# zhiqwang/demonet

Measured on AMD Instinct MI355X. Metric: images/sec ssdlite320_mobilenet_v3_large fp16 end-to-end incl. NMS, higher is better.
Workload: dtype fp16; 1 GPU; ssdlite320_mobilenet_v3_large fp16, batch 64 per GPU, 320x320 synthetic images, K=91, synthetic weights seed 0, post-process incl. per-class top-300 + hard NMS; global_batch=64, forwards_in_flight=3, parallelism=single GPU, input=NCHW fp32 in [0,1], device-resident

## Files before the change

demonet_amd/csrc/headfuse.hip:

```cpp
#include <algorithm>
#include <type_traits>

#include "common.h"
#include "post_math.h"

namespace {

constexpr int HF_P = 64;
constexpr int HF_RUNP = 128;
constexpr int HF_ZOFF = 4 * HF_RUNP * 16;
constexpr int HF_WOFF = HF_ZOFF + 64;
constexpr int HF_XS = HF_WOFF + 1024;
constexpr int HF_BS = 4 * HF_P * 16;
constexpr int HF_LDS = 2 * HF_XS + 4 * HF_BS;
constexpr int HF_NP = 2;
constexpr int hf_post_tabs(int nc0, int nc1) {
    const int t = 32 * (nc0 + nc1) * 4 + 3 * 256 * 4 + HF_NP * 256 * 4 + 256;
    return t > HF_LDS ? t : HF_LDS;
}
constexpr int hf_post_lds(int nc0, int nc1) { return hf_post_tabs(nc0, nc1) + (((nc0 + 3) & ~3) + ((nc1 + 3) & ~3)) * 4; }

typedef unsigned u32x4 __attribute__((ext_vector_type(4)));
typedef unsigned u32x8 __attribute__((ext_vector_type(8)));
typedef float f32x8 __attribute__((ext_vector_type(8)));
typedef float f32x4_a8 __attribute__((ext_vector_type(4), aligned(8)));
typedef unsigned u32x16 __attribute__((ext_vector_type(16)));
typedef const __attribute__((address_space(4))) u32x4* cp_u4;
typedef const __attribute__((address_space(4))) u32x16* cp_u16;

struct HfLevel {
    const half_t* x;
    const half_t* wd;
    const unsigned char* wslot;
    const half_t* wf[2];
    const float* bias[2];
    float* out[2];
    unsigned out_img_stride[2];
    int nc[2];
    int H, W, C, hw, m;
    int act;
    int tiles;
    int ct0;
    int aoff, aloc, sbase;
    int sm;
};
struct HfGroup {
    int count, xq;
    int start[9];
    long long* stamps;
    HeadPost post;
    HfLevel lv[8];
};
#ifdef DN_DEV_STAMPS
#define HF_T(var) const long long var = (long long)__builtin_amdgcn_s_memtime()
#else
#define HF_T(var)
#endif

__device__ __forceinline__ void hf_fma8(float (&acc)[8], const u32x4& x, const u32x4& w) {
#pragma unroll
    for (int i = 0; i < 4; ++i) {
        asm("v_fma_mix_f32 %0, %1, %2, %0 op_sel_hi:[1,1,0]" : "+v"(acc[2 * i]) : "v"(x[i]), "s"(w[i]));
        asm("v_fma_mix_f32 %0, %1, %2, %0 op_sel:[1,1,0] op_sel_hi:[1,1,0]" : "+v"(acc[2 * i + 1]) : "v"(x[i]), "s"(w[i]));
    }
}

__device__ __forceinline__ void hf_fma8v(float (&acc)[8], const u32x4& x, const u32x4& w) {
#pragma unroll
    for (int i = 0; i < 4; ++i) {
        asm("v_fma_mix_f32 %0, %1, %2, %0 op_sel_hi:[1,1,0]" : "+v"(acc[2 * i]) : "v"(x[i]), "v"(w[i]));
        asm("v_fma_mix_f32 %0, %1, %2, %0 op_sel:[1,1,0] op_sel_hi:[1,1,0]" : "+v"(acc[2 * i + 1]) : "v"(x[i]), "v"(w[i]));
    }
}

constexpr int HF_SM_BATCHES = 3;
constexpr int HF_SM_MAX_K = 4 * 8 * HF_SM_BATCHES;
static_assert(HF_SM_MAX_K == 96, "hf_softmax_scores covers 96 classes: change head_fused_post_supported's bound with it");
__device__ __forceinline__ void hf_softmax_scores(const HeadPost& P, const float* __restrict__ lg, const unsigned* __restrict__ rowoff, const unsigned* __restrict__ ranc,
                                                  const unsigned char* __restrict__ rpart, unsigned* __restrict__ lhist, const int nrows, const int img_first,
                                                  const int te, const int K, const int ccb) {
#pragma clang fp contract(off)
    const int Km1 = K - 1, sub = te & 3;
    char* const sbase = reinterpret_cast<char*>(P.scoresT);
    const unsigned step4 = 4u * (unsigned)P.A;
    for (int rb = 0; rb < nrows; rb += 64) {
        const int row = rb + (te >> 2);
        const bool valid = row < nrows;
        const float* rp = lg + (valid ? rowoff[row] : 0u);
        float mx = -INFINITY, sm = 0.f;
        float v[8 * HF_SM_BATCHES];
#pragma unroll
        for (int b = 0; b < HF_SM_BATCHES; ++b) {
#pragma unroll
            for (int u = 0; u < 8; ++u) v[8 * b + u] = rp[min(sub + 32 * b + 4 * u, K - 1)];
#pragma unroll
            for (int u = 0; u < 8; ++u) mx = fmaxf(mx, v[8 * b + u]);
        }
        mx = fmaxf(mx, __shfl_xor(mx, 1));
        mx = fmaxf(mx, __shfl_xor(mx, 2));
#pragma unroll
        for (int b = 0; b < HF_SM_BATCHES; ++b) {
#pragma unroll
            for (int u = 0; u < 8; ++u) v[8 * b + u] = pp_exp_nonpos(v[8 * b + u] - mx);
#pragma unroll
            for (int u = 0; u < 8; ++u)
                if (sub + 32 * b + 4 * u < K) sm += v[8 * b + u];
        }
        sm += __shfl_xor(sm, 1);
        sm += __shfl_xor(sm, 2);
        if (!valid) continue;
        const float rinv = pp_row_rcp(sm);
        int rw = row;
        asm volatile("" : "+v"(rw));
        const unsigned q = rpart[rw];
        const unsigned hb = q * 256u;
        const unsigned ob4 = (((unsigned)(img_first + (int)q) * (unsigned)Km1) * (unsigned)P.A + ranc[rw]) * 4u + (unsigned)(sub - 1) * step4;
#pragma unroll
        for (int b = 0; b < HF_SM_BATCHES; ++b)
#pragma unroll
            for (int u = 0; u < 8; ++u) {
                const int k = sub + 32 * b + 4 * u;
                if (k >= 1 && k < K) {
                    const float sc = pp_score(v[8 * b + u], rinv);
                    *reinterpret_cast<float*>(sbase + (unsigned)(ob4 + (unsigned)(8 * b + u) * 4u * step4)) = sc;
                    if (sc > P.score_thr) {
                        atomicAdd(&lhist[hb + (unsigned)pp_hist_bin(sc, P.hb0, P.nb)], 1u);
                        if (ccb >= 0) atomicAdd(&lhist[hb + (unsigned)(ccb + k - 1)], 1u);
                    }
                }
            }
    }
}

template <int TCW, bool SM>
__global__ __launch_bounds__(256, 2) void head_fused_kernel(HfGroup g) {
    extern __shared__ __attribute__((aligned(16))) unsigned char hf_lds[];
    int p = 0;
#pragma unroll
    for (int i = 1; i < 8; ++i)
        if (i < g.count && (int)blockIdx.x >= g.start[i]) p = i;
    const HfLevel& L = g.lv[p];
    const int flat = blockIdx.x - g.start[p];
    int m0, mend;
    if (g.xq > 0 && L.tiles > 0) {
        const int grp = flat & 7, t = flat >> 3;
        const int r0 = grp * g.xq * L.hw;
        mend = min(L.m, r0 + g.xq * L.hw);
        m0 = r0 + t * HF_P;
    } else {
        m0 = flat * HF_P;
        mend = L.m;
    }
    if (m0 >= mend) return;

    const int tid = threadIdx.x, lane = tid & 63;
    const int wave = __builtin_amdgcn_readfirstlane(tid >> 6);
    const int r = lane & 31, hh = lane >> 5;
    const int C = L.C, W = L.W, H = L.H;
    const int NCH = C >> 5;

    unsigned tap3[3] = {0u, 0u, 0u};
    {
        const int mp = min(m0 + lane, mend - 1);
        const int img = mp / L.hw, rem = mp - img * L.hw;
        const int y = rem / W, x = rem - y * W;
#pragma unroll
        for (int ky = 0; ky < 3; ++ky)
#pragma unroll
            for (int kx = 0; kx < 3; ++kx) {
                const int iy = y + ky - 1, ix = x + kx - 1;
                const bool ok = iy >= 0 && iy < H && ix >= 0 && ix < W;
                const int P = lane + (W + 1) + (ky - 1) * W + (kx - 1);
                const unsigned slot = ok ? (unsigned)(4 * P + (wave ^ ((P >> 2) & 3))) : (unsigned)(HF_ZOFF / 16);
                tap3[ky] |= slot << (10 * kx);
            }
    }
    auto tap_addr = [&](int t) -> unsigned { return ((tap3[t / 3] >> (10 * (t % 3))) & 1023u) * 16u; };
    unsigned xoff[2];
#pragma unroll
    for (int i = 0; i < 2; ++i) {
        const int P = (2 * wave + i) * 16 + (lane >> 2);
        const int mp = min(max(m0 - (W + 1) + P, 0), L.m - 1);
        xoff[i] = ((unsigned)mp * (unsigned)C + (unsigned)(((lane & 3) ^ ((P >> 2) & 3)) * 8)) * 2u;
    }
    if (tid < 8) *reinterpret_cast<unsigned*>(hf_lds + (tid >> 2) * HF_XS + HF_ZOFF + (tid & 3) * 4) = 0u;
    const unsigned lds0 = (unsigned)(size_t)(__attribute__((address_space(3))) unsigned char*)hf_lds;
    auto glds16 = [&](const void* gsrc, unsigned dst) {
        unsigned keep;
        asm volatile("s_mov_b32 %0, m0\n\ts_mov_b32 m0, %2\n\ts_nop 0\n\tglobal_load_lds_dwordx4 %1, off\n\ts_mov_b32 m0, %0"
                     : "=&s"(keep) : "v"(gsrc), "s"(dst) : "memory");
    };
    const unsigned aoff = (unsigned)lane * 16u;
    const unsigned char* const xbase = reinterpret_cast<const unsigned char*>(L.x);
    auto stage_x = [&](int c) {
        const unsigned dst = lds0 + (c & 1) * HF_XS;
        glds16(xbase + (xoff[0] + (unsigned)c * 64u), dst + wave * 2048);
        glds16(xbase + (xoff[1] + (unsigned)c * 64u), dst + wave * 2048 + 1024);
        if (wave == 3) glds16(L.wslot + ((unsigned)c * 1024u + aoff), dst + HF_WOFF);
    };

    const int tlast = wave + 4 * (TCW - 1);
    const bool last_reg = tlast == L.ct0, last_on = tlast <= L.ct0;
    const int KS = C >> 4;
    const __amdgpu_buffer_rsrc_t ars0 = __builtin_amdgcn_make_buffer_rsrc(const_cast<half_t*>(L.wf[0]), 0, L.ct0 * KS * 1024, 0x00020000);
    const __amdgpu_buffer_rsrc_t ars1 = __builtin_amdgcn_make_buffer_rsrc(const_cast<half_t*>(L.wf[1]), 0, KS * 1024, 0x00020000);
    unsigned atile[TCW];
#pragma unroll
    for (int i = 0; i < TCW; ++i) {
        const int t = wave + 4 * i;
        const bool reg = (i == TCW - 1) && last_reg;
        atile[i] = reg ? 0u : (unsigned)(min(t, L.ct0 - 1) * KS) * 1024u;
    }
    auto load_a = [&](int i, int kstep) -> half8 {
        const u32x4 v = ((i == TCW - 1) && last_reg) ? __builtin_amdgcn_raw_buffer_load_b128(ars1, aoff, atile[i] + (unsigned)kstep * 1024u, 0)
                                                     : __builtin_amdgcn_raw_buffer_load_b128(ars0, aoff, atile[i] + (unsigned)kstep * 1024u, 0);
        return __builtin_bit_cast(half8, v);
    };
    const unsigned blast = last_reg ? (unsigned)HF_BS : 0u;

    floatx16 acc[TCW][2];
#pragma unroll
    for (int i = 0; i < TCW; ++i)
#pragma unroll
        for (int j = 0; j < 2; ++j)
#pragma unroll
            for (int e = 0; e < 16; ++e) acc[i][j][e] = 0.f;

    u32x16 w0a, w0b;
    u32x4 w0c;
    auto load_w0 = [&](int c) {
        const unsigned char* wp = reinterpret_cast<const unsigned char*>(L.wd) + (size_t)(c * 4 + wave) * 144;
        w0a = *(cp_u16)(wp);
        w0b = *(cp_u16)(wp + 64);
        w0c = *(cp_u4)(wp + 128);
    };
    auto w0tap = [&](int t) -> u32x4 {
        u32x4 r;
#pragma unroll
        for (int e = 0; e < 4; ++e) { const int d = 4 * t + e; r[e] = d < 16 ? w0a[d] : (d < 32 ? w0b[d - 16] : w0c[d - 32]); }
        return r;
    };

#ifdef DN_DEV_STAMPS
    long long st_dw = 0, st_wait = 0, st_mm = 0;
    const long long st_begin = (long long)__builtin_amdgcn_s_memtime();
    const long long st_begin_rt = (long long)__builtin_amdgcn_s_memrealtime();
#endif
    if constexpr (SM) if (L.sm) {
        float* const lb = reinterpret_cast<float*>(hf_lds + hf_post_tabs(L.nc[0], L.nc[1]));
        const int p0 = (L.nc[0] + 3) & ~3;
        for (int i = tid; i < L.nc[0]; i += 256) lb[i] = L.bias[0][i];
        if (tid < L.nc[1]) lb[p0 + tid] = L.bias[1][tid];
    }
    stage_x(0);
    load_w0(0);
    asm volatile("s_waitcnt vmcnt(0)" ::: "memory");
    __syncthreads();
    HF_T(st_loop);

    unsigned char* const bb = hf_lds + 2 * HF_XS;
    for (int c = 0; c < NCH; ++c) {
        const int PAR = c & 1;
        HF_T(st0);
        half8 af0[TCW], af1[TCW];
#pragma unroll
        for (int i = 0; i < TCW; ++i) af0[i] = load_a(i, 2 * c);
        {
            const unsigned char* xb = hf_lds + PAR * HF_XS;
            const unsigned char* wb = xb + HF_WOFF + wave * 144;
            asm volatile("" : "+v"(tap3[0]), "+v"(tap3[1]), "+v"(tap3[2]));
            const float4 bl4 = *reinterpret_cast<const float4*>(xb + HF_WOFF + 576 + wave * 32);
            const float4 bh4 = *reinterpret_cast<const float4*>(xb + HF_WOFF + 576 + wave * 32 + 16);
            const float4 cl4 = *reinterpret_cast<const float4*>(xb + HF_WOFF + 704 + wave * 32);
            const float4 ch4 = *reinterpret_cast<const float4*>(xb + HF_WOFF + 704 + wave * 32 + 16);
            float a0[8] = {cl4.x, cl4.y, cl4.z, cl4.w, ch4.x, ch4.y, ch4.z, ch4.w}, a1[8] = {bl4.x, bl4.y, bl4.z, bl4.w, bh4.x, bh4.y, bh4.z, bh4.w};
#pragma unroll
            for (int ky = 0; ky < 3; ++ky) {
                u32x4 tap[3], wv[3];
#pragma unroll
                for (int kx = 0; kx < 3; ++kx) {
                    tap[kx] = *reinterpret_cast<const u32x4*>(xb + tap_addr(ky * 3 + kx));
                    wv[kx] = *reinterpret_cast<const u32x4*>(wb + (ky * 3 + kx) * 16);
                }
                if (ky == 0 && c + 1 < NCH) stage_x(c + 1);
#pragma unroll
                for (int kx = 0; kx < 3; ++kx) hf_fma8(a0, tap[kx], w0tap(ky * 3 + kx));
                if (ky == 2) {
#pragma unroll
                    for (int i = 0; i < TCW; ++i) af1[i] = load_a(i, 2 * c + 1);
                }
#pragma unroll
                for (int kx = 0; kx < 3; ++kx) hf_fma8v(a1, tap[kx], wv[kx]);
                __builtin_amdgcn_sched_barrier(0);
            }
            unsigned char* bout = bb + PAR * 2 * HF_BS + wave * (HF_P * 16) + lane * 16;
            half8 o0, o1;
#pragma unroll
            for (int e = 0; e < 8; ++e) { o0[e] = (half_t)dn_relu6(a0[e]); o1[e] = (half_t)dn_relu6(a1[e]); }
            *reinterpret_cast<half8*>(bout) = o0;
            *reinterpret_cast<half8*>(bout + HF_BS) = o1;
        }
        HF_T(st1);
        asm volatile("s_waitcnt vmcnt(%0)" :: "n"(TCW) : "memory");
        __syncthreads();
        HF_T(st2);
        load_w0(min(c + 1, NCH - 1));
        {
            const unsigned char* bc = bb + PAR * 2 * HF_BS;
#pragma unroll
            for (int s = 0; s < 2; ++s) {
                half8 bf[2];
#pragma unroll
                for (int j = 0; j < 2; ++j) bf[j] = *reinterpret_cast<const half8*>(bc + (unsigned)((2 * s + hh) * (HF_P * 16) + (32 * j + r) * 16));
#pragma unroll
                for (int i = 0; i < TCW - 1; ++i)
#pragma unroll
                    for (int j = 0; j < 2; ++j) acc[i][j] = __builtin_amdgcn_mfma_f32_32x32x16_f16(s ? af1[i] : af0[i], bf[j], acc[i][j], 0, 0, 0);
                if (last_on) {
#pragma unroll
                    for (int j = 0; j < 2; ++j) {
                        const half8 bl = *reinterpret_cast<const half8*>(bc + blast + (unsigned)((2 * s + hh) * (HF_P * 16) + (32 * j + r) * 16));
                        acc[TCW - 1][j] = __builtin_amdgcn_mfma_f32_32x32x16_f16(s ? af1[TCW - 1] : af0[TCW - 1], bl, acc[TCW - 1][j], 0, 0, 0);
                    }
                }
            }
        }
#ifdef DN_DEV_STAMPS
        asm volatile("" : "+v"(acc[0][0]));
        const long long st3 = (long long)__builtin_amdgcn_s_memtime();
        st_dw += st1 - st0; st_wait += st2 - st1; st_mm += st3 - st2;
#endif
    }
#ifdef DN_DEV_STAMPS
    const long long st_end_loop = (long long)__builtin_amdgcn_s_memtime();
#endif
    int te = threadIdx.x;
    if constexpr (SM) asm volatile("" : "+v"(te));
    const int lane_e = SM ? (te & 63) : lane, r_e = SM ? (lane_e & 31) : r, hh_e = SM ? (lane_e >> 5) : hh;
    if constexpr (SM) if (L.sm) {
        const HeadPost& P = g.post;
        const int lane = lane_e, r = r_e, hh = hh_e;
        const int K = P.K, Km1 = K - 1, AL = L.aloc, NC0 = L.nc[0], NC1 = L.nc[1], hw = L.hw;
        float* const lg = reinterpret_cast<float*>(hf_lds);
        float* const rgt = lg + 32 * NC0;
        float* const rowsum = rgt + 32 * NC1;
        unsigned* const rowoff = reinterpret_cast<unsigned*>(rowsum + 256);
        unsigned* const ranc = rowoff + 256;
        unsigned* const lhist = ranc + 256;
        unsigned char* const rpart = reinterpret_cast<unsigned char*>(lhist + HF_NP * 256);
        const int ccb = (P.nb + Km1 <= 256) ? P.nb : -1;
        const bool grouped = g.xq > 0 && L.tiles > 0;
        const int img_g0 = grouped ? (flat & 7) * g.xq : 0;
        const int r0 = img_g0 * hw;
        __syncthreads();
#ifdef DN_DEV_STAMPS
        long long st_w = 0, st_s = 0, st_p = 0;
#endif
#pragma unroll
        for (int j = 0; j < 2; ++j) {
            const int mj = m0 + 32 * j;
            if (mj >= mend) break;
            HF_T(se0);
            const int npx = min(32, mend - mj), nrows = npx * AL;
            const int img_first = mj / hw, img_last = (mj + npx - 1) / hw;
#pragma unroll
            for (int i = 0; i < TCW; ++i) {
                const bool reg = (i == TCW - 1) && last_reg;
                if (i == TCW - 1 && !last_on) break;
                const int ct = reg ? 0 : wave + 4 * i;
                const int nc = reg ? NC1 : NC0;
                const float* bias = reinterpret_cast<const float*>(hf_lds + hf_post_tabs(NC0, NC1)) + (reg ? ((NC0 + 3) & ~3) : 0);
                float* drow = (reg ? rgt : lg) + r * nc;
#pragma unroll
                for (int gq = 0; gq < 4; ++gq) {
                    const int ch = 32 * ct + 8 * gq + 4 * hh;
                    const float4 b4 = *reinterpret_cast<const float4*>(bias + min(ch, ((nc + 3) & ~3) - 4));
                    const float v[4] = {acc[i][j][4 * gq] + b4.x, acc[i][j][4 * gq + 1] + b4.y, acc[i][j][4 * gq + 2] + b4.z, acc[i][j][4 * gq + 3] + b4.w};
                    if (ch + 4 <= nc) {
                        *reinterpret_cast<float2*>(drow + ch) = make_float2(v[0], v[1]);
                        *reinterpret_cast<float2*>(drow + ch + 2) = make_float2(v[2], v[3]);
                    } else if (ch + 2 <= nc) {
                        *reinterpret_cast<float2*>(drow + ch) = make_float2(v[0], v[1]);
                    }
                }
            }
            for (int t = te; t < HF_NP * 256; t += 256) lhist[t] = 0u;
            int bx_px = 0, bx_a = 0, bx_img = 0, bx_anc = 0;
            if (te < nrows) {
                bx_px = te / AL; bx_a = te - bx_px * AL;
                const int m = mj + bx_px;
                bx_img = m / hw;
                bx_anc = L.aoff + (m - bx_img * hw) * AL + bx_a;
                rowoff[te] = (unsigned)(bx_px * NC0 + bx_a * K);
                ranc[te] = (unsigned)bx_anc;
                rpart[te] = (unsigned char)(bx_img - img_first);
            }
            __syncthreads();
            HF_T(se1);
            if (te < nrows) {
                const float4 rg4 = *reinterpret_cast<const float4*>(rgt + bx_px * NC1 + bx_a * 4);
                const float4 an = reinterpret_cast<const float4*>(P.anchors)[bx_anc];
                P.boxes[(size_t)bx_img * P.A + bx_anc] = pp_decode_box(rg4, an, P.img_w, P.img_h);
            }
            hf_softmax_scores(P, lg, rowoff, ranc, rpart, lhist, nrows, img_first, te, K, ccb);
            __syncthreads();
            HF_T(se2);
#pragma unroll
            for (int qq = 0; qq < HF_NP; ++qq) {
                const int img = img_first + qq;
                if (img <= img_last) {
                    const int slot = ((mj - r0) >> 5) - (((img - img_g0) * hw) >> 5);
                    P.hrows[((size_t)img * P.rows_per_image + L.sbase + slot) * 256 + te] = (te < P.nb + (ccb >= 0 ? Km1 : 0)) ? lhist[qq * 256 + te] : 0u;
                }
            }
            __syncthreads();
#ifdef DN_DEV_STAMPS
            const long long se3 = (long long)__builtin_amdgcn_s_memtime();
            st_w += se1 - se0; st_s += se2 - se1; st_p += se3 - se2;
#endif
        }
#ifdef DN_DEV_STAMPS
        if (g.stamps && te == 0) {
            long long* sp = g.stamps + (size_t)blockIdx.x * 16;
            sp[8] = st_begin_rt;
            sp[9] = (long long)__builtin_amdgcn_s_getreg((4 << 0) | (0 << 6) | (31 << 11));
            sp[10] = (long long)__builtin_amdgcn_s_getreg((20 << 0) | (0 << 6) | (31 << 11));
            sp[0] = st_loop - st_begin; sp[1] = st_dw; sp[2] = st_wait; sp[3] = st_mm; sp[4] = st_end_loop - st_loop;
            sp[5] = (long long)__builtin_amdgcn_s_memtime() - st_end_loop; sp[6] = NCH; sp[7] = (long long)__builtin_amdgcn_s_memrealtime();
            sp[11] = st_w; sp[12] = st_s; sp[13] = st_p;
        }
#endif
        return;
    }
    unsigned ro[2][2];
    bool rok[2];
#pragma unroll
    for (int j = 0; j < 2; ++j) {
        const int m = m0 + 32 * j + r_e;
        const int img = m / L.hw, pix = m - img * L.hw;
        rok[j] = m < mend;
#pragma unroll
        for (int h = 0; h < 2; ++h) ro[h][j] = (unsigned)img * L.out_img_stride[h] + (unsigned)pix * (unsigned)L.nc[h];
    }
#pragma unroll
    for (int i = 0; i < TCW; ++i) {
        const bool reg = (i == TCW - 1) && last_reg;
        if (i == TCW - 1 && !last_on) break;
        const int ct = reg ? 0 : wave + 4 * i;
        const int nc = reg ? L.nc[1] : L.nc[0];
        const float* bias = reg ? L.bias[1] : L.bias[0];
        float* outp = reg ? L.out[1] : L.out[0];
        float bv[16];
#pragma unroll
        for (int gq = 0; gq < 4; ++gq)
#pragma unroll
            for (int e = 0; e < 4; ++e) bv[4 * gq + e] = bias[min(32 * ct + 8 * gq + 4 * hh_e + e, nc - 1)];
#pragma unroll
        for (int j = 0; j < 2; ++j) {
            float* orow = outp + (reg ? ro[1][j] : ro[0][j]);
#pragma unroll
            for (int gq = 0; gq < 4; ++gq) {
                const int ch = 32 * ct + 8 * gq + 4 * hh_e;
                floatx4 v;
#pragma unroll
                for (int e = 0; e < 4; ++e) v[e] = acc[i][j][4 * gq + e] + bv[4 * gq + e];
                if (rok[j]) {
                    if (ch + 4 <= nc) *reinterpret_cast<f32x4_a8*>(orow + ch) = v;
                    else if (ch + 2 <= nc) *reinterpret_cast<float2*>(orow + ch) = make_float2(v[0], v[1]);
                }
            }
        }
    }
#ifdef DN_DEV_STAMPS
    if (g.stamps && tid == 0) {
        long long* sp = g.stamps + (size_t)blockIdx.x * 16;
        sp[8] = st_begin_rt;
        sp[9] = (long long)__builtin_amdgcn_s_getreg((4 << 0) | (0 << 6) | (31 << 11));
        sp[10] = (long long)__builtin_amdgcn_s_getreg((20 << 0) | (0 << 6) | (31 << 11));
        sp[0] = st_loop - st_begin; sp[1] = st_dw; sp[2] = st_wait; sp[3] = st_mm; sp[4] = st_end_loop - st_loop;
        sp[5] = (long long)__builtin_amdgcn_s_memtime() - st_end_loop; sp[6] = NCH; sp[7] = (long long)__builtin_amdgcn_s_memrealtime();
    }
#endif
}

}

bool head_fused_level_supported(const HeadFuseLevel& l) {
    if (l.C % 32 != 0 || l.C < 32 || l.W > 31 || l.W < 1 || l.H < 1 || l.act != DN_ACT_RELU6) return false;
    if (l.nc[1] > 32 || l.nc[0] < 1 || l.nc[1] < 1 || !l.wdg || !l.wslot) return false;
    for (int h = 0; h < 2; ++h) {
        if ((l.nc[h] & 1) || (l.out_img_stride[h] & 1) || (l.out_base[h] & 1) || (reinterpret_cast<size_t>(l.out[h]) & 7)) return false;
        if ((unsigned long long)l.n * (unsigned long long)l.out_img_stride[h] >= 0xffffffffull) return false;
        if (!l.wf[h] || !l.bias[h]) return false;
    }
    const int tiles = dn_cdiv(l.nc[0], 32) + 1;
    return dn_cdiv(tiles, 4) <= 5 && (unsigned long long)l.n * l.H * l.W * l.C < 0x80000000ull;
}

#ifdef DN_DEV_STAMPS
static long long* g_hf_stamps = nullptr;
extern "C" __attribute__((visibility("default"))) void dn_debug_hf_stamps(void* dev_ptr) { g_hf_stamps = (long long*)dev_ptr; }
#endif
static int g_head_fused_launches = 0, g_head_softmax_launches = 0;
extern "C" __attribute__((visibility("default"))) int dn_debug_head_fused_launches() { return g_head_fused_launches; }
extern "C" __attribute__((visibility("default"))) int dn_debug_head_softmax_launches() { return g_head_softmax_launches; }

bool head_fused_post_supported(const HeadFuseLevel* lv, int count, const HeadPost& post) {
    if (!post.scoresT || !post.boxes || !post.hrows || !post.anchors || post.K < 2 || post.A < 1 || post.nb < 1 || post.nb > 256) return false;
    if (post.K > HF_SM_MAX_K) return false;
    int rows = 0, nsm = 0;
    for (int i = 0; i < count; ++i) {
        const HeadFuseLevel& l = lv[i];
        if (!l.sm) continue;
        ++nsm;
        if (l.H * l.W < 32) return false;
        if (l.aloc < 1 || l.aloc > 8 || l.nc[0] != l.aloc * post.K || l.nc[1] != 4 * l.aloc) return false;
        if (hf_post_lds(l.nc[0], l.nc[1]) > 80 * 1024) return false;
        if (l.sbase != rows) return false;
        rows += hist_rows_slots(l.H * l.W);
        if ((unsigned long long)l.n * (post.K - 1) * post.A >= 0x3fffffffull) return false;
    }
    return nsm > 0 && rows <= post.rows_per_image;
}

int launch_head_fused(const HeadFuseLevel* lv, int count, int xq, hipStream_t s, const HeadPost* post) {
    DN_REQUIRE(count >= 1 && count <= 8, "fused heads: %d levels", count);
    HfGroup g{};
    g.count = count; g.xq = xq;
    int lds = HF_LDS;
    if (post) {
        DN_REQUIRE(head_fused_post_supported(lv, count, *post), "fused heads: softmax epilogue not supported for these levels");
        g.post = *post;
        for (int i = 0; i < count; ++i)
            if (lv[i].sm) lds = std::max(lds, hf_post_lds(lv[i].nc[0], lv[i].nc[1]));
    }
    int ord[8];
    for (int i = 0; i < count; ++i) ord[i] = i;
    if (post)
        std::stable_sort(ord, ord + count, [&](int x, int y) {
            if (lv[x].sm != lv[y].sm) return lv[x].sm > lv[y].sm;
            return lv[x].sm ? lv[x].C > lv[y].C : false;
        });
    int acc = 0, tcw = 0;
    for (int i = 0; i < count; ++i) {
        const HeadFuseLevel& l = lv[ord[i]];
        DN_REQUIRE(head_fused_level_supported(l), "fused heads: level %d unsupported (C=%d W=%d nc=%d/%d)", ord[i], l.C, l.W, l.nc[0], l.nc[1]);
        HfLevel& d = g.lv[i];
        d.x = l.x; d.wd = l.wdg; d.wslot = l.wslot;
        for (int h = 0; h < 2; ++h) {
            d.wf[h] = l.wf[h]; d.bias[h] = l.bias[h];
            d.out[h] = l.out[h] + l.out_base[h];
            d.out_img_stride[h] = (unsigned)l.out_img_stride[h];
            d.nc[h] = l.nc[h];
        }
        d.H = l.H; d.W = l.W; d.C = l.C; d.hw = l.H * l.W; d.m = l.n * d.hw; d.act = l.act;
        d.ct0 = dn_cdiv(l.nc[0], 32);
        d.aoff = l.aoff; d.aloc = l.aloc; d.sbase = l.sbase; d.sm = post ? l.sm : 0;
        const int t4 = dn_cdiv(d.ct0 + 1, 4);
        DN_REQUIRE(i == 0 || t4 == tcw, "fused heads: levels differ in channel tiles per wave (%d vs %d)", t4, tcw);
        tcw = t4;
        const bool grouped = head_fused_grouped(xq, d.hw);
        d.tiles = grouped ? dn_cdiv((long)xq * d.hw, HF_P) : 0;
        g.start[i] = acc;
        acc += grouped ? d.tiles * 8 : dn_cdiv(d.m, HF_P);
    }
    g.start[count] = acc;
#ifdef DN_DEV_STAMPS
    g.stamps = g_hf_stamps;
#endif
    dn_note_kernel(post ? "head_fused_kernel<%d,softmax>" : "head_fused_kernel<%d>", tcw);
    ++g_head_fused_launches;
    if (post) ++g_head_softmax_launches;
    const dim3 grid(acc), block(256);
#define HF_GO(T)                                                                                                            \
    if (post) {                                                                                                             \
        DN_HIP_CHECK(dn_allow_big_lds(reinterpret_cast<const void*>(head_fused_kernel<T, true>), 160 * 1024));               \
        hipLaunchKernelGGL((head_fused_kernel<T, true>), grid, block, lds, s, g);                                           \
    } else {                                                                                                                \
        if (lds > 64 * 1024) DN_HIP_CHECK(dn_allow_big_lds(reinterpret_cast<const void*>(head_fused_kernel<T, false>), 160 * 1024)); \
        hipLaunchKernelGGL((head_fused_kernel<T, false>), grid, block, lds, s, g);                                          \
    }
    switch (tcw) {
        case 1: HF_GO(1); break;
        case 2: HF_GO(2); break;
        case 3: HF_GO(3); break;
        case 4: HF_GO(4); break;
        case 5: HF_GO(5); break;
        default: DN_REQUIRE(false, "fused heads: %d channel tiles per wave", tcw);
    }
#undef HF_GO
    return DN_OK;
}
```

Baseline: 107,300 images/sec.

## Coalesce softmax score stores into 16-byte writes via DPP quad transpose

In the fused head softmax epilogue, each thread used to write transposed class scores as scattered 4-byte stores. Now, when four consecutive rows belong to the same image, each group of four lanes transposes its scores with DPP row-rotate operations so every lane writes one 16-byte vector, cutting the number of global store instructions. The post-processing parameters are also reloaded late from the kernarg segment with explicit global address spaces, which should lower SGPR/VGPR pressure in the main loop. This adds DPP shuffle work and a runtime knob (on by default), and assumes the ranc values of the four rows are contiguous.

```diff
diff --git a/demonet_amd/csrc/headfuse.hip b/demonet_amd/csrc/headfuse.hip
--- a/demonet_amd/csrc/headfuse.hip
+++ b/demonet_amd/csrc/headfuse.hip
@@ -1,4 +1,5 @@
 #include <algorithm>
+#include <cstddef>
 #include <type_traits>
 
 #include "common.h"
@@ -24,9 +25,12 @@
 typedef unsigned u32x8 __attribute__((ext_vector_type(8)));
 typedef float f32x8 __attribute__((ext_vector_type(8)));
 typedef float f32x4_a8 __attribute__((ext_vector_type(4), aligned(8)));
+typedef float f32x4_a4 __attribute__((ext_vector_type(4), aligned(4)));
 typedef unsigned u32x16 __attribute__((ext_vector_type(16)));
 typedef const __attribute__((address_space(4))) u32x4* cp_u4;
 typedef const __attribute__((address_space(4))) u32x16* cp_u16;
+typedef const __attribute__((address_space(4))) unsigned char* cp_u8;
+typedef __attribute__((address_space(1))) char* gp_c8;
 
 struct HfLevel {
     const half_t* x;
@@ -49,6 +53,7 @@
     int start[9];
     long long* stamps;
     HeadPost post;
+    int store16;
     HfLevel lv[8];
 };
 #ifdef DN_DEV_STAMPS
@@ -76,12 +81,33 @@
 constexpr int HF_SM_BATCHES = 3;
 constexpr int HF_SM_MAX_K = 4 * 8 * HF_SM_BATCHES;
 static_assert(HF_SM_MAX_K == 96, "hf_softmax_scores covers 96 classes: change head_fused_post_supported's bound with it");
-__device__ __forceinline__ void hf_softmax_scores(const HeadPost& P, const float* __restrict__ lg, const unsigned* __restrict__ rowoff, const unsigned* __restrict__ ranc,
-                                                  const unsigned char* __restrict__ rpart, unsigned* __restrict__ lhist, const int nrows, const int img_first,
-                                                  const int te, const int K, const int ccb) {
+
+template <typename T>
+__device__ __forceinline__ T hf_karg(cp_u8 ka, const size_t off) { return *reinterpret_cast<const __attribute__((address_space(4))) T*>(ka + off); }
+__device__ __forceinline__ cp_u8 hf_late_kargs() {
+    cp_u8 ka = (cp_u8)__builtin_amdgcn_kernarg_segment_ptr();
+    asm volatile("" : "+s"(ka));
+    return ka;
+}
+
+template <int ROR, int BANK>
+__device__ __forceinline__ float hf_ror_bank(const float own, const float src) {
+    return __builtin_bit_cast(float, __builtin_amdgcn_update_dpp(__builtin_bit_cast(int, own), __builtin_bit_cast(int, src), 0x120 + ROR, 0xf, 1 << BANK, false));
+}
+__device__ __forceinline__ void hf_transpose4(float (&t)[4]) {
+    const float a0 = t[0], a1 = t[1], a2 = t[2], a3 = t[3];
+    t[0] = hf_ror_bank<4, 1>(a0, a1); t[0] = hf_ror_bank<8, 2>(t[0], a2); t[0] = hf_ror_bank<12, 3>(t[0], a3);
+    t[1] = hf_ror_bank<4, 2>(a1, a2); t[1] = hf_ror_bank<8, 3>(t[1], a3); t[1] = hf_ror_bank<12, 0>(t[1], a0);
+    t[2] = hf_ror_bank<4, 3>(a2, a3); t[2] = hf_ror_bank<8, 0>(t[2], a0); t[2] = hf_ror_bank<12, 1>(t[2], a1);
+    t[3] = hf_ror_bank<4, 0>(a3, a0); t[3] = hf_ror_bank<8, 1>(t[3], a1); t[3] = hf_ror_bank<12, 2>(t[3], a2);
+}
+
+__device__ __forceinline__ void hf_softmax_scores(const HeadPost& P, const bool store16, const float* __restrict__ lg, const unsigned* __restrict__ rowoff,
+                                                  const unsigned* __restrict__ ranc, const unsigned char* __restrict__ rpart, unsigned* __restrict__ lhist,
+                                                  const int nrows, const int img_first, const int te, const int K, const int ccb) {
 #pragma clang fp contract(off)
     const int Km1 = K - 1, sub = te & 3;
-    char* const sbase = reinterpret_cast<char*>(P.scoresT);
+    const gp_c8 sbase = (gp_c8)P.scoresT;
     const unsigned step4 = 4u * (unsigned)P.A;
     for (int rb = 0; rb < nrows; rb += 64) {
         const int row = rb + (te >> 2);
@@ -114,7 +140,12 @@
         asm volatile("" : "+v"(rw));
         const unsigned q = rpart[rw];
         const unsigned hb = q * 256u;
-        const unsigned ob4 = (((unsigned)(img_first + (int)q) * (unsigned)Km1) * (unsigned)P.A + ranc[rw]) * 4u + (unsigned)(sub - 1) * step4;
+        int sb = rw * 4 + sub;
+        asm volatile("" : "+v"(sb));
+        const int subs = sb & 3, bank = (sb >> 2) & 3;
+        const unsigned img_col = (unsigned)(img_first + (int)q) * (unsigned)Km1 * (unsigned)P.A;
+        const int r4 = rw & ~3;
+        const bool quad = store16 && r4 + 3 < nrows && rpart[r4 + 3] == rpart[r4];
 #pragma unroll
         for (int b = 0; b < HF_SM_BATCHES; ++b)
 #pragma unroll
@@ -122,13 +153,38 @@
                 const int k = sub + 32 * b + 4 * u;
                 if (k >= 1 && k < K) {
                     const float sc = pp_score(v[8 * b + u], rinv);
-                    *reinterpret_cast<float*>(sbase + (unsigned)(ob4 + (unsigned)(8 * b + u) * 4u * step4)) = sc;
+                    v[8 * b + u] = sc;
                     if (sc > P.score_thr) {
                         atomicAdd(&lhist[hb + (unsigned)pp_hist_bin(sc, P.hb0, P.nb)], 1u);
                         if (ccb >= 0) atomicAdd(&lhist[hb + (unsigned)(ccb + k - 1)], 1u);
                     }
                 }
             }
+        if (quad) {
+            const unsigned ob4 = (img_col + ranc[r4]) * 4u + (unsigned)(subs + 4 * bank - 1) * step4;
+#pragma unroll
+            for (int b = 0; b < HF_SM_BATCHES; ++b)
+#pragma unroll
+                for (int u0 = 0; u0 < 8; u0 += 4) {
+                    float t[4] = {v[8 * b + u0], v[8 * b + u0 + 1], v[8 * b + u0 + 2], v[8 * b + u0 + 3]};
+                    hf_transpose4(t);
+                    const int k = subs + 32 * b + 4 * (u0 + bank);
+                    if (k >= 1 && k < K) {
+                        f32x4_a4 o;
+                        o[0] = t[0]; o[1] = t[1]; o[2] = t[2]; o[3] = t[3];
+                        *(__attribute__((address_space(1))) f32x4_a4*)(sbase + (unsigned)(ob4 + (unsigned)(32 * b + 4 * u0) * step4)) = o;
+                    }
+                }
+        } else {
+            const unsigned ob4 = (img_col + ranc[rw]) * 4u + (unsigned)(subs - 1) * step4;
+#pragma unroll
+            for (int b = 0; b < HF_SM_BATCHES; ++b)
+#pragma unroll
+                for (int u = 0; u < 8; ++u) {
+                    const int k = subs + 32 * b + 4 * u;
+                    if (k >= 1 && k < K) *(__attribute__((address_space(1))) float*)(sbase + (unsigned)(ob4 + (unsigned)(8 * b + u) * 4u * step4)) = v[8 * b + u];
+                }
+        }
     }
 }
 
@@ -338,7 +394,18 @@
     if constexpr (SM) asm volatile("" : "+v"(te));
     const int lane_e = SM ? (te & 63) : lane, r_e = SM ? (lane_e & 31) : r, hh_e = SM ? (lane_e >> 5) : hh;
     if constexpr (SM) if (L.sm) {
-        const HeadPost& P = g.post;
+        const cp_u8 ka = hf_late_kargs();
+        HeadPost P;
+        P.scoresT = reinterpret_cast<float*>(hf_karg<unsigned long long>(ka, offsetof(HfGroup, post.scoresT)));
+        P.boxes = reinterpret_cast<float4*>(hf_karg<unsigned long long>(ka, offsetof(HfGroup, post.boxes)));
+        P.hrows = reinterpret_cast<unsigned*>(hf_karg<unsigned long long>(ka, offsetof(HfGroup, post.hrows)));
+        P.anchors = reinterpret_cast<const float*>(hf_karg<unsigned long long>(ka, offsetof(HfGroup, post.anchors)));
+        P.A = hf_karg<int>(ka, offsetof(HfGroup, post.A)); P.K = hf_karg<int>(ka, offsetof(HfGroup, post.K));
+        P.rows_per_image = hf_karg<int>(ka, offsetof(HfGroup, post.rows_per_image));
+        P.hb0 = hf_karg<int>(ka, offsetof(HfGroup, post.hb0)); P.nb = hf_karg<int>(ka, offsetof(HfGroup, post.nb));
+        P.img_w = hf_karg<float>(ka, offsetof(HfGroup, post.img_w)); P.img_h = hf_karg<float>(ka, offsetof(HfGroup, post.img_h));
+        P.score_thr = hf_karg<float>(ka, offsetof(HfGroup, post.score_thr));
+        const bool store16 = hf_karg<int>(ka, offsetof(HfGroup, store16)) != 0;
         const int lane = lane_e, r = r_e, hh = hh_e;
         const int K = P.K, Km1 = K - 1, AL = L.aloc, NC0 = L.nc[0], NC1 = L.nc[1], hw = L.hw;
         float* const lg = reinterpret_cast<float*>(hf_lds);
@@ -399,10 +466,13 @@
             HF_T(se1);
             if (te < nrows) {
                 const float4 rg4 = *reinterpret_cast<const float4*>(rgt + bx_px * NC1 + bx_a * 4);
-                const float4 an = reinterpret_cast<const float4*>(P.anchors)[bx_anc];
-                P.boxes[(size_t)bx_img * P.A + bx_anc] = pp_decode_box(rg4, an, P.img_w, P.img_h);
-            }
-            hf_softmax_scores(P, lg, rowoff, ranc, rpart, lhist, nrows, img_first, te, K, ccb);
+                const floatx4 an4 = ((const __attribute__((address_space(1))) floatx4*)P.anchors)[bx_anc];
+                const float4 bx = pp_decode_box(rg4, make_float4(an4[0], an4[1], an4[2], an4[3]), P.img_w, P.img_h);
+                floatx4 bx4;
+                bx4[0] = bx.x; bx4[1] = bx.y; bx4[2] = bx.z; bx4[3] = bx.w;
+                ((__attribute__((address_space(1))) floatx4*)P.boxes)[(size_t)bx_img * P.A + bx_anc] = bx4;
+            }
+            hf_softmax_scores(P, store16, lg, rowoff, ranc, rpart, lhist, nrows, img_first, te, K, ccb);
             __syncthreads();
             HF_T(se2);
 #pragma unroll
@@ -410,7 +480,7 @@
                 const int img = img_first + qq;
                 if (img <= img_last) {
                     const int slot = ((mj - r0) >> 5) - (((img - img_g0) * hw) >> 5);
-                    P.hrows[((size_t)img * P.rows_per_image + L.sbase + slot) * 256 + te] = (te < P.nb + (ccb >= 0 ? Km1 : 0)) ? lhist[qq * 256 + te] : 0u;
+                    ((__attribute__((address_space(1))) unsigned*)P.hrows)[((size_t)img * P.rows_per_image + L.sbase + slot) * 256 + te] = (te < P.nb + (ccb >= 0 ? Km1 : 0)) ? lhist[qq * 256 + te] : 0u;
                 }
             }
             __syncthreads();
@@ -531,6 +601,7 @@
     if (post) {
         DN_REQUIRE(head_fused_post_supported(lv, count, *post), "fused heads: softmax epilogue not supported for these levels");
         g.post = *post;
+        g.store16 = dn_knob("DN_HEAD_STORE16", 1) != 0;
         for (int i = 0; i < count; ++i)
             if (lv[i].sm) lds = std::max(lds, hf_post_lds(lv[i].nc[0], lv[i].nc[1]));
     }
```

After: 106,800 images/sec. No clear change (-0.4%).
